# Wuziyi616/LEOD

Hardware: AMD Instinct MI355X
Metric: event-frames/sec/GPU (RVT-S train, Gen1 T=21) at 1/2/4/8 GPUs; mAP@0.5 parity (higher is better)
Workload: dtype fp16

## Files before the change

leod_amd/csrc/k_linear_wgrad.hip:

```cpp
#include "linear_common.hpp"
#include "wgrad_bf16.hpp"
#include "wgrad_dma.hpp"

LEOD_API long leod_workspace_bytes() { return (long)kWgwScratchBytes; }
LEOD_API int leod_set_workspace(void* ws, long bytes, hipStream_t stream) {
    if (ws && (bytes <= 0 || (reinterpret_cast<uintptr_t>(ws) & 15))) return LEOD_ERR_ARG;
    wgrad_wide_register_scratch(stream, ws, (size_t)(bytes > 0 ? bytes : 0));
    return LEOD_OK;
}

__global__ void leod_family_marker_kernel(int begin) { (void)begin; }
struct FamilyMarker {
    hipStream_t s; bool on;
    explicit FamilyMarker(hipStream_t st) : s(st) {
        static const bool env = getenv("LEOD_FAMILY_MARKERS") && atoi(getenv("LEOD_FAMILY_MARKERS"));
        on = env;
        if (on) hipLaunchKernelGGL(leod_family_marker_kernel, dim3(1), dim3(1), 0, s, 1);
    }
    ~FamilyMarker() { if (on) hipLaunchKernelGGL(leod_family_marker_kernel, dim3(1), dim3(1), 0, s, 0); }
};

enum : int { WGR_NONE = 0, WGR_DMA = 100, WGR_WIDE = 200, WGR_WGRADW = 300, WGR_LADDER = 400 };
static int wgrad_route(const XRows& xl, long lddy, int dyfmt, int M, int N, int K, bool dma = true) {
    const int xm = xl.x_mode();
    const bool x16 = xm == XM_BF16 || xm == XM_F16;
    if (x16 && (xl.stats || xl.x2)) return LEOD_ERR_ARG;
    if (dma && wgrad_dma_ok(xl, lddy, M, N, K, dyfmt)) return WGR_DMA + wgd_tile(N, K);
    if (use_wgrad_wide(xl, lddy, M, N, K, dyfmt)) return WGR_WIDE + wgrad_wide_combo(xl, N, K, dyfmt);
    if (x16) return LEOD_ERR_UNSUPPORTED;
    if (M <= 0) return WGR_NONE;
    if (!wgrad_rows16b_ok(lddy, N, K)) return LEOD_ERR_ARG;
// ... 98 lines not shown
```

leod_amd/csrc/wgrad_bf16.hpp:

```cpp
#pragma once

typedef unsigned u4_ __attribute__((ext_vector_type(4)));

__device__ __forceinline__ f2_ gelu_erf2(f2_ x) {
    const f2_ z = __builtin_elementwise_abs(x) * 0.70710678118654752440f;
    const f2_ d = z * 0.3275911f + 1.0f;
    const f2_ t = {fast_rcp(d.x), fast_rcp(d.y)};
    const f2_ poly = t * (0.254829592f + t * (-0.284496736f + t * (1.421413741f + t * (-1.453152027f + t * 1.061405429f))));
    const f2_ a = (z * z) * -1.4426950408889634f;
    const f2_ e = {__builtin_amdgcn_exp2f(a.x), __builtin_amdgcn_exp2f(a.y)};
    const f2_ ht = (0.5f * poly) * e;
    const f2_ cdf = {x.x >= 0.f ? 1.0f - ht.x : ht.x, x.y >= 0.f ? 1.0f - ht.y : ht.y};
    return x * cdf;
}
__device__ __forceinline__ unsigned pack_bf16x2(f2_ v) { return __builtin_bit_cast(unsigned, __builtin_convertvector(v, bf2_)); }

constexpr int wgw_row_groups(int slots_per_row) {
    int g = 1;
    while (2 * g * slots_per_row <= 256) g *= 2;
    return g;
}
template <int RG, int T, int BST>
__device__ __forceinline__ constexpr int wgw_slot_off(int e) {
    return RG >= 16 ? e * (RG / 16) * T * BST : (e % (16 / (RG < 16 ? RG : 16))) * RG * 16 + (e / (16 / (RG < 16 ? RG : 16))) * T * BST;
}

template <int TN, int TK, int RC, int MS = 1>
constexpr int wgw_lds_bytes() {
    return 2 * ((RC / 16) * (TN + TK) * 272) * 2 > (MS - 1) * 12 * 1024 ? 2 * ((RC / 16) * (TN + TK) * 272) * 2 : (MS - 1) * 12 * 1024;
}

template <int TN, int TK, int NWN, int NWK, int RC, int DYF, int XM, int OCC>
__global__ __launch_bounds__(256, OCC) void wgrad_wide_bf16_kernel(const void* __restrict__ dyv, long lddy, XRows xl, float* dW, long ldw,
                                                                    float* dbias, f4* __restrict__ part, int M, int N, int K, int dbg) {
    constexpr int WA = TN / NWN, WB = TK / NWK, MS = 4 / (NWN * NWK), KS = RC / 32;
    constexpr bool K16 = KS % MS != 0;
    constexpr int NSL = WA * WB + WA;
    static_assert((WA == 3 || WA == 6) && (WB == 3 || WB == 6) && WA * WB <= 18 && NWN * NWK * MS == 4 && (RC / 16) % MS == 0 &&
                  (MS == 1 || (WA == 3 && WB == 3)), "4 waves of 3 x 3, 6 x 3 or 3 x 6 tiles");
    constexpr int BST = 16 * 16 + 16;
    constexpr int DCW = DYF ? 8 : 4, XCW = XM >= XM_GELU16 ? 8 : 4;
    constexpr int DSPR = 16 * TN / DCW, XSPR = 16 * TK / XCW;
    constexpr int DRG = wgw_row_groups(DSPR) < RC ? wgw_row_groups(DSPR) : RC, XRG = wgw_row_groups(XSPR) < RC ? wgw_row_groups(XSPR) : RC;
    constexpr bool XG = XM == XM_GELU16;
    static_assert(!XG || (RC * XSPR) % 256 == 0, "whole slots per thread");
    constexpr int RN = RC / DRG, RK = XG ? RC * XSPR / 256 : RC / XRG;
    constexpr int SDY = (RC / 16) * TN * BST, SX = (RC / 16) * TK * BST;
    static_assert(DSPR * DRG == 192 && (XG || XSPR * XRG == 192), "three waves stage an operand");
    static_assert(2 * (SDY + SX) * 2 <= wgw_lds_bytes<TN, TK, RC, MS>(), "LDS size");
    extern __shared__ __attribute__((aligned(16))) unsigned short wg_smem[];
    const int tid = threadIdx.x, lane = tid & 63, wave = __builtin_amdgcn_readfirstlane(tid >> 6);
    const int i = lane & 15, q = lane >> 4;
    const int wn = wave % NWN, wk = (wave / NWN) % NWK, ws = wave / (NWN * NWK);
    const int n0 = blockIdx.y * TN * 16, k0 = blockIdx.z * TK * 16;
    const bool dact = wave < 3, xact = XG || wave >= 1;
    const int xt = tid - 64;
    const int dcs = tid % DSPR, drg = tid / DSPR, xcs = (xact ? xt : 0) % XSPR, xrg = (xact ? xt : 0) / XSPR;
// ... 186 lines not shown
    }
    __syncthreads();
    int buf = 0;
    for (; m0 < M; m0 += mstride) {
        const long mn = m0 + mstride;
        const bool more = mn < M;
        if (more) { if (mn + RC <= M) fetch(mn, FULL); else fetch(mn, TAILC); }
        if (!(dbg & 2)) mfma_chunk(buf);
        if (more) stash(mn, buf ^ 1);
        __syncthreads();
        buf ^= 1;
    }
    if constexpr (MS > 1) {
        f4* sred = reinterpret_cast<f4*>(wg_smem);
        if (ws > 0) {
#pragma unroll
            for (int a = 0; a < WA; ++a) {
#pragma unroll
                for (int b = 0; b < WB; ++b) sred[((ws - 1) * NSL + a * WB + b) * 64 + lane] = acc[a][b];
                sred[((ws - 1) * NSL + WA * WB + a) * 64 + lane] = bacc[a];
            }
        }
        __syncthreads();
        if (ws > 0) return;
#pragma unroll
        for (int o = 0; o < MS - 1; ++o)
#pragma unroll
            for (int a = 0; a < WA; ++a) {
#pragma unroll
                for (int b = 0; b < WB; ++b) acc[a][b] += sred[(o * NSL + a * WB + b) * 64 + lane];
                bacc[a] += sred[(o * NSL + WA * WB + a) * 64 + lane];
            }
    }
    if (dbg & 1) return;
    if constexpr (XM == XM_LN) {
#pragma unroll
        for (int b = 0; b < WB; ++b) {
            const int k = k0 + 16 * (wk * WB + b) + i;
            const float g = k < K ? xl.ln_w[k] : 0.f, sh = k < K ? xl.ln_b[k] : 0.f;
#pragma unroll
            for (int a = 0; a < WA; ++a)
#pragma unroll
                for (int r = 0; r < 4; ++r) acc[a][b][r] = fmaf(g, acc[a][b][r], sh * bacc[a][r]);
        }
    }
    const bool bias_out = dbias != nullptr && blockIdx.z == 0;
    if (part != nullptr) {
        constexpr int NW = NWN * NWK;
        const long tile = (long)blockIdx.y * gridDim.z + blockIdx.z, ntiles = (long)gridDim.y * gridDim.z;
        f4* dst = part + (((long)blockIdx.x * ntiles + tile) * NW + (wk * NWN + wn)) * (NSL * 64) + lane;
#pragma unroll
        for (int a = 0; a < WA; ++a) {
#pragma unroll
            for (int b = 0; b < WB; ++b) dst[(a * WB + b) * 64] = acc[a][b];
            if (bias_out && a % NWK == wk) dst[(WA * WB + a) * 64] = bacc[a];
        }
        return;
    }
#pragma unroll
    for (int b = 0; b < WB; ++b) {
        const int k = k0 + 16 * (wk * WB + b) + i;
#pragma unroll
        for (int a = 0; a < WA; ++a)
#pragma unroll
            for (int r = 0; r < 4; ++r) {
                const int n = n0 + 16 * (wn * WA + a) + 4 * q + r;
                if (n < N && k < K) atomicAdd(dW + (long)n * ldw + k, acc[a][b][r]);
            }
    }
    if (bias_out && i == 0) {
#pragma unroll
        for (int a = 0; a < WA; ++a)
            if (a % NWK == wk) {
#pragma unroll
                for (int r = 0; r < 4; ++r) {
                    const int n = n0 + 16 * (wn * WA + a) + 4 * q + r;
                    if (n < N) atomicAdd(dbias + n, bacc[a][r]);
                }
            }
    }
}

template <int TN, int TK, int NWN, int NWK>
__global__ __launch_bounds__(256) void wgrad_wide_reduce_kernel(const f4* __restrict__ part, int gx, int ny, int nz, int per, float* dW, long ldw,
                                                                float* dbias, int N, int K) {
    constexpr int NW = NWN * NWK, WA = TN / NWN, WB = TK / NWK, NT9 = WA * WB, NSL = NT9 + WA;
    const long O = (long)ny * nz * NW * NSL * 64;
    const long o = (long)blockIdx.x * 256 + threadIdx.x;
    if (o >= O) return;
    const int lane = (int)(o & 63), t = (int)((o >> 6) % NSL), w = (int)((o / (64 * NSL)) % NW), tile = (int)(o / (64 * NSL * NW));
    const int ty = tile / nz, tz = tile - ty * nz, wn = w % NWN, wk = w / NWN, i = lane & 15, q = lane >> 4;
    if (t >= NT9 && !(dbias != nullptr && tz == 0 && (t - NT9) % NWK == wk && i == 0)) return;
    const int g0 = blockIdx.y * per, g1 = min(gx, g0 + per);
    f4 s0 = zero4(), s1 = zero4(), s2 = zero4(), s3 = zero4();
    const f4* p = part + (long)g0 * O + o;
    int g = g0;
    f4 s4 = zero4(), s5 = zero4(), s6 = zero4(), s7 = zero4();
    for (; g + 8 <= g1; g += 8, p += 8 * O) {
        s0 += p[0]; s1 += p[O]; s2 += p[2 * O]; s3 += p[3 * O]; s4 += p[4 * O]; s5 += p[5 * O]; s6 += p[6 * O]; s7 += p[7 * O];
    }
    for (; g + 4 <= g1; g += 4, p += 4 * O) { s0 += p[0]; s1 += p[O]; s2 += p[2 * O]; s3 += p[3 * O]; }
    for (; g < g1; ++g, p += O) s0 += p[0];
    const f4 v = ((s0 + s1) + (s2 + s3)) + ((s4 + s5) + (s6 + s7));
    const bool single = gridDim.y == 1;
    if (t < NT9) {
        const int a = t / WB, b = t - a * WB;
        const int k = tz * TK * 16 + 16 * (wk * WB + b) + i;
#pragma unroll
        for (int r = 0; r < 4; ++r) {
            const int n = ty * TN * 16 + 16 * (wn * WA + a) + 4 * q + r;
            if (n < N && k < K) {
                float* d = dW + (long)n * ldw + k;
                if (single) *d += v[r]; else atomicAdd(d, v[r]);
            }
        }
    } else {
#pragma unroll
        for (int r = 0; r < 4; ++r) {
            const int n = ty * TN * 16 + 16 * (wn * WA + (t - NT9)) + 4 * q + r;
            if (n < N) { if (single) dbias[n] += v[r]; else atomicAdd(dbias + n, v[r]); }
        }
    }
}

#include <mutex>
#include <unordered_map>
struct WgwScratch { void* p = nullptr; size_t bytes = 0; };
static inline std::unordered_map<hipStream_t, WgwScratch>& wgw_scratch_map() { static std::unordered_map<hipStream_t, WgwScratch> m; return m; }
static inline std::mutex& wgw_scratch_mutex() { static std::mutex m; return m; }
constexpr size_t kWgwScratchBytes = (size_t)768 << 20;
static inline void wgrad_wide_register_scratch(hipStream_t s, void* p, size_t bytes) {
    std::lock_guard<std::mutex> lock(wgw_scratch_mutex());
    WgwScratch& e = wgw_scratch_map()[s];
    e.p = p; e.bytes = p ? bytes : 0;
}
static inline f4* wgrad_wide_scratch(hipStream_t s, size_t bytes) {
    std::lock_guard<std::mutex> lock(wgw_scratch_mutex());
    WgwScratch& e = wgw_scratch_map()[s];
    if (e.bytes >= bytes) return reinterpret_cast<f4*>(e.p);
    hipStreamCaptureStatus cs = hipStreamCaptureStatusNone;
    if (hipStreamIsCapturing(s, &cs) != hipSuccess || cs != hipStreamCaptureStatusNone) { (void)hipGetLastError(); return nullptr; }
    void* nb = nullptr;
    const size_t want = bytes < kWgwScratchBytes ? kWgwScratchBytes : bytes;
    if (hipMalloc(&nb, want) != hipSuccess) { (void)hipGetLastError(); return nullptr; }
    e.p = nb; e.bytes = want;
    return reinterpret_cast<f4*>(nb);
}

template <int TN, int TK, int NWN, int NWK, int RC, int DYF, int XM, int OCC>
static inline int launch_wgrad_wide_cfg(const void* dy, long lddy, const XRows& xl, float* dW, long ldw, float* dbias,
                                        int M, int N, int K, hipStream_t s) {
    constexpr int dbg = 0;
    constexpr int LDS = wgw_lds_bytes<TN, TK, RC, 4 / (NWN * NWK)>();
    const int tiles = cdiv(N, TN * 16) * cdiv(K, TK * 16), chunks = cdiv(M, RC);
    const int wgs = M <= 60000 ? 384 : OCC * 256;
    int gx = max(1, min(chunks / 2, wgs / tiles));
    if (gx >= 16) gx &= ~7;
    dim3 grid(gx, cdiv(N, TN * 16), cdiv(K, TK * 16));
    auto kern = wgrad_wide_bf16_kernel<TN, TK, NWN, NWK, RC, DYF, XM, OCC>;
    static bool attr_set = false;
    if (!attr_set) { hipFuncSetAttribute(reinterpret_cast<const void*>(kern), hipFuncAttributeMaxDynamicSharedMemorySize, LDS); attr_set = true; }
    constexpr int NW = NWN * NWK, NSL = (TN / NWN) * (TK / NWK) + TN / NWN;
    const long O = (long)tiles * NW * NSL * 64;
    f4* part = gx > 1 ? wgrad_wide_scratch(s, (size_t)gx * O * sizeof(f4)) : nullptr;
    hipLaunchKernelGGL(kern, grid, dim3(256), LDS, s, dy, lddy, xl, dW, ldw, dbias, part, M, N, K, dbg);
    if (part != nullptr && !(dbg & 1)) {
        const int ob = (int)cdiv(O, 256);
        int groups = max(1, min(gx, 512 / ob));
        const int per = cdiv(gx, groups);
        groups = cdiv(gx, per);
        hipLaunchKernelGGL((wgrad_wide_reduce_kernel<TN, TK, NWN, NWK>), dim3(ob, groups), dim3(256), 0, s, part, gx, (int)grid.y, (int)grid.z, per,
                           dW, ldw, dbias, N, K);
    }
    return leod_launch_status();
}

static inline int wgrad_wide_combo(const XRows& xl, int N, int K, int dyfmt) {
    const int xm = xl.x_mode();
    if (xm == XM_F16) {
        if (dyfmt) return 0;
        if (N <= 48 && K <= 48) return 14;
        if (K <= 48 || N <= 48) return 0;
        return (K % 192 == 0 && N >= 96) ? 16 : 15;
    }
    const bool f32_rows = !dyfmt && xm == XM_ROWS, f32_gelu = !dyfmt && xm == XM_GELU16, f32_bf16 = !dyfmt && xm == XM_BF16;
    const bool b16_rows = dyfmt && xm == XM_ROWS, b16_ln = dyfmt && xm == XM_LN;
    if (N <= 48 && K <= 48) return f32_rows ? 1 : f32_bf16 ? 8 : 0;
    if (K <= 48) return b16_ln ? 2 : 0;
    if (N <= 48) return f32_gelu ? 3 : 0;
    if (N % 192 == 0 && K >= 96 && (b16_ln || b16_rows)) return b16_ln ? 10 : 11;
    if (K % 192 == 0 && N >= 96 && (f32_gelu || f32_bf16)) return f32_gelu ? 12 : 13;
    return f32_rows ? 4 : b16_ln ? 5 : f32_gelu ? 6 : b16_rows ? 7 : f32_bf16 ? 9 : 0;
}
static inline bool use_wgrad_wide(const XRows& xl, long lddy, int M, int N, int K, int dyfmt) {
    if (leod_precision() != 1 || M < 8192) return false;
    const int xm = xl.x_mode();
// ... 31 lines not shown
```

leod_amd/csrc/wgrad_dma.hpp:

```cpp
#pragma once

struct Prep16 {
    const void* src; long ld;
    const float* src2; long ld2; int C1;
    const float* stats;
    unsigned short* dst;
    int C, mode;
};
enum Prep16Mode : int { P16_NONE = -1, P16_F32 = 0, P16_LN = 1 , P16_GELU16 = 2, P16_F16 = 3, P16_CONCAT = 4  };
static inline int prep16_mode(int xm, bool concat) {
    if (xm_is_mfma_operand(xm)) return P16_NONE;
    return xm == XM_LN ? P16_LN : xm == XM_GELU16 ? P16_GELU16 : xm == XM_F16 ? P16_F16 : concat ? P16_CONCAT : P16_F32;
}

struct Prep16Group { Prep16 a[4]; Prep16 b[4]; };
__global__ __launch_bounds__(256) void wgrad_prep16_kernel(Prep16Group grp, int M) {
    const Prep16& p = blockIdx.y ? grp.b[blockIdx.z] : grp.a[blockIdx.z];
    if (p.mode < 0) return;
    const int C8 = p.C >> 3;
    const long it = (long)blockIdx.x * 256 + threadIdx.x;
    if (it >= (long)M * C8) return;
    const long m = it / C8;
    const int c = (int)(it - m * C8) << 3;
    f4 lo, hi;
// ... 6 lines not shown
    } else {
        const float* s = (p.mode == 4 && c >= p.C1) ? p.src2 + m * p.ld2 + (c - p.C1) : reinterpret_cast<const float*>(p.src) + m * p.ld + c;
        lo = ld4(s); hi = ld4(s + 4);
        if (p.mode == 1) {
            const f2_ st = *reinterpret_cast<const f2_*>(p.stats + 2 * m);
            lo = (lo - st.x) * st.y; hi = (hi - st.x) * st.y;
        }
    }
    const u4_ o = {pack_bf16x2(f2_{lo.x, lo.y}), pack_bf16x2(f2_{lo.z, lo.w}), pack_bf16x2(f2_{hi.x, hi.y}), pack_bf16x2(f2_{hi.z, hi.w})};
    *reinterpret_cast<u4_*>(p.dst + m * p.C + c) = o;
}

__device__ __forceinline__ void wgd_dma16(const void* gsrc, unsigned lds_dst) {
    unsigned keep;
    asm volatile("s_mov_b32 %0, m0\n\ts_mov_b32 m0, %2\n\ts_nop 0\n\tglobal_load_lds_dwordx4 %1, off\n\ts_mov_b32 m0, %0"
                 : "=&s"(keep) : "v"(gsrc), "s"(lds_dst) : "memory");
}
template <int N> __device__ __forceinline__ void wgd_wait_vm() { asm volatile("s_waitcnt vmcnt(%0)" :: "n"(N) : "memory"); }

template <int T, int RC, int NS> constexpr int wgd_lds_bytes() { return NS * 2 * (RC / 16) * T * 256 * 2; }
template <int T, int RC, int NS> constexpr int wgd_occupancy() { return wgd_lds_bytes<T, RC, NS>() <= 52 * 1024 ? 3 : wgd_lds_bytes<T, RC, NS>() <= 80 * 1024 ? 2 : 1; }

struct WgdProb {
    const unsigned short* A; long lda; const unsigned short* B; long ldb; const float* ln_w; const float* ln_b; float* dbias_flag; f4* part;
    int cpw, gx, ny, nz, N, K, blk0;
};
struct WgdGroup { WgdProb p[4]; int n; };
template <int T, int RC, int NS, bool LN>
__global__ __launch_bounds__(256, ((wgd_occupancy<T, RC, NS>()) >= 2 ? 2 : 1)) void wgrad_dma_kernel(WgdGroup grp, int chunks, int dbg) {
    int pk = 0;
    for (int k = 1; k < grp.n; ++k) if ((int)blockIdx.x >= grp.p[k].blk0) pk = k;
    const WgdProb& pr = grp.p[pk];
    const unsigned short* __restrict__ A = pr.A; const unsigned short* __restrict__ B = pr.B; const long lda = pr.lda, ldb = pr.ldb;
    const float* __restrict__ ln_w = pr.ln_w; const float* __restrict__ ln_b = pr.ln_b; float* dbias_flag = pr.dbias_flag; f4* __restrict__ part = pr.part;
    const int cpw = pr.cpw, gx = pr.gx, ny = pr.ny, nz = pr.nz, K = pr.K;
    const int bid = (int)blockIdx.x - pr.blk0;
    const bool ln = LN && ln_w != nullptr;
    constexpr int WA = T / 2, WB = T / 2, NWN = 2, NWK = 2, RB = RC / 16, KS = RC / 32;
    constexpr int BLK = 256;
    constexpr int SA = RB * T * BLK, SLOT = 2 * SA;
    constexpr int NI = SLOT * 2 / 1024, IPW = NI / 4;
    static_assert(NI % 4 == 0 && RC % 32 == 0, "whole instructions per wave");
    constexpr int NSL = WA * WB + WA;
    extern __shared__ __attribute__((aligned(1024))) unsigned short wd_smem[];
    const int tid = threadIdx.x, lane = tid & 63, wave = __builtin_amdgcn_readfirstlane(tid >> 6);
    const int i = lane & 15, q = lane >> 4;
    const int wn = wave % NWN, wk = wave / NWN;
    const int ntl = ny * nz;
    int tl, bx;
    if ((gx & 7) == 0) { const int xcd = bid & 7, sj = bid >> 3; tl = sj % ntl; bx = (sj / ntl) * 8 + xcd; }
    else { bx = bid % gx; tl = bid / gx; }
    const int by = tl / nz, bz = tl - by * nz;
    const int n0 = by * T * 16, k0 = bz * T * 16;
    const int c0 = bx * cpw, c1 = min(chunks, c0 + cpw);
    const int nch = c1 - c0;
    static_assert(IPW % 2 == 0, "the first half of a wave's instructions fills the dY part, the second half the X part");
    const char* src[IPW];
    const long stepA = (long)RC * lda * 2, stepB = (long)RC * ldb * 2;
#pragma unroll
    for (int j = 0; j < IPW; ++j) {
        const int t = wave + 4 * j;
        const int blk = 2 * t + (lane >> 5), r = (lane & 31) >> 1, half = lane & 1;
        const bool isb = j >= IPW / 2;
        const int b = isb ? blk - RB * T : blk;
        const int rb = b / T, cb = b - rb * T;
        const long ld = isb ? ldb : lda;
        const int col = (isb ? k0 : n0) + cb * 16 + half * 8;
        src[j] = reinterpret_cast<const char*>(isb ? B : A) + (((long)c0 * RC + rb * 16 + r) * ld + col) * 2;
    }
    const unsigned lds0 = __builtin_amdgcn_readfirstlane((unsigned)(size_t)wd_smem);
    auto issue = [&](int slot) {
#pragma unroll
        for (int j = 0; j < IPW; ++j) {
            wgd_dma16(src[j], __builtin_amdgcn_readfirstlane(lds0 + (unsigned)(slot * SLOT * 2 + (wave + 4 * j) * 1024)));
            src[j] += j >= IPW / 2 ? stepB : stepA;
        }
    };
    const bool bias_out = dbias_flag != nullptr && bz == 0;
    const bool bias_any = ln || bias_out;
    f4 acc[WA][WB], bacc[WA];
#pragma unroll
    for (int a = 0; a < WA; ++a) {
        bacc[a] = zero4();
#pragma unroll
        for (int b = 0; b < WB; ++b) acc[a][b] = zero4();
    }
    const s8v ones = {0x3F80, 0x3F80, 0x3F80, 0x3F80, 0x3F80, 0x3F80, 0x3F80, 0x3F80};
    typedef __attribute__((address_space(3))) s4 lds_s4;
    const int loff = (4 * q + (i >> 2)) * 16 + 4 * (i & 3);
    auto mfma_chunk = [&](int slot) {
        const unsigned short* pdy = wd_smem + slot * SLOT + (wn * WA) * BLK + loff;
        const unsigned short* px = wd_smem + slot * SLOT + SA + (wk * WB) * BLK + loff;
#pragma unroll
        for (int ks = 0; ks < KS; ++ks) {
            const int st = 2 * ks;
            s8v pa[WA], pb[WB];
#pragma unroll
            for (int a = 0; a < WA; ++a) {
                const s4 lo = __builtin_amdgcn_ds_read_tr16_b64_v4i16((lds_s4*)(pdy + (st * T + a) * BLK));
                const s4 hi = __builtin_amdgcn_ds_read_tr16_b64_v4i16((lds_s4*)(pdy + ((st + 1) * T + a) * BLK));
                pa[a] = __builtin_shufflevector(lo, hi, 0, 1, 2, 3, 4, 5, 6, 7);
// ... 25 lines not shown
        if (c + NS - 1 < nch && !(dbg & 2)) issue((c + NS - 1) % NS);
        if (!(dbg & 1)) mfma_chunk(c % NS);
    }
    if (ln) {
#pragma unroll
        for (int b = 0; b < WB; ++b) {
            const int k = k0 + 16 * (wk * WB + b) + i;
            const float g = k < K ? ln_w[k] : 0.f, sh = k < K ? ln_b[k] : 0.f;
#pragma unroll
            for (int a = 0; a < WA; ++a)
#pragma unroll
                for (int r = 0; r < 4; ++r) acc[a][b][r] = fmaf(g, acc[a][b][r], sh * bacc[a][r]);
        }
    }
    constexpr int NW = NWN * NWK;
    const long tile = (long)by * nz + bz, ntiles = ntl;
    f4* dst = part + (((long)bx * ntiles + tile) * NW + (wk * NWN + wn)) * (NSL * 64) + lane;
#pragma unroll
    for (int a = 0; a < WA; ++a) {
#pragma unroll
        for (int b = 0; b < WB; ++b) dst[(a * WB + b) * 64] = acc[a][b];
        if (bias_out && a % NWK == wk) dst[(WA * WB + a) * 64] = bacc[a];
    }
}

constexpr int kWgdRC = 64;
constexpr size_t kWgdOperandBytes = (size_t)600 << 20;

static inline int wgd_tile(int N, int K) {
    if (N % 96 == 0 && K % 96 == 0) return 6;
    if (N % 128 == 0 && K % 128 == 0) return 8;
    if (N % 64 == 0 && K % 64 == 0) return 4;
    return 0;
}
static inline bool wgrad_dma_ok(const XRows& xl, long lddy, int M, int N, int K, int dyfmt) {
    if (leod_precision() != 1 || M < 8192 || (M % kWgdRC) || N < 64 || K < 64) return false;
    const int T = wgd_tile(N, K);
    if (!T) return false;
    const int xm = xl.x_mode();
    if ((lddy & 7) || (xl.ld & 7)) return false;
    if (xl.x2 && (xm != XM_ROWS || (xl.K1 & 7) || (xl.ld2 & 7))) return false;
    const size_t need = (size_t)M * ((dyfmt ? 0 : N) + (xm_is_mfma_operand(xm) ? 0 : K)) * 2;
    if (need > kWgdOperandBytes) return false;
    if (M > (T == 6 ? 60000 : 400000)) return false;
    if (!dyfmt && xm != XM_BF16 && xm != XM_GELU16 && (long)N * K < 200000) return false;
    return true;
}

struct WgrProb { const f4* part; float* dW; float* dbias; long ldw; int gx, ny, nz, per, N, K, ob, groups; };
struct WgrGroup { WgrProb p[4]; };
template <int T>
__global__ __launch_bounds__(256) void wgrad_dma_reduce_kernel(WgrGroup grp) {
    const WgrProb& pr = grp.p[blockIdx.z];
    if ((int)blockIdx.x >= pr.ob || (int)blockIdx.y >= pr.groups) return;
    constexpr int NWN = 2, NWK = 2, NW = 4, WA = T / 2, WB = T / 2, NT9 = WA * WB, NSL = NT9 + WA;
    const int gx = pr.gx, nz = pr.nz, per = pr.per, N = pr.N, K = pr.K;
    float* dW = pr.dW; float* dbias = pr.dbias; const long ldw = pr.ldw;
    const long O = (long)pr.ny * nz * NW * NSL * 64;
    const long o = (long)blockIdx.x * 256 + threadIdx.x;
    if (o >= O) return;
    const int lane = (int)(o & 63), t = (int)((o >> 6) % NSL), w = (int)((o / (64 * NSL)) % NW), tile = (int)(o / (64 * NSL * NW));
    const int ty = tile / nz, tz = tile - ty * nz, wn = w % NWN, wk = w / NWN, i = lane & 15, q = lane >> 4;
    if (t >= NT9 && !(dbias != nullptr && tz == 0 && (t - NT9) % NWK == wk && i == 0)) return;
    const int g0 = blockIdx.y * per, g1 = min(gx, g0 + per);
    f4 s0 = zero4(), s1 = zero4(), s2 = zero4(), s3 = zero4(), s4 = zero4(), s5 = zero4(), s6 = zero4(), s7 = zero4();
    const f4* p = pr.part + (long)g0 * O + o;
    int g = g0;
    for (; g + 8 <= g1; g += 8, p += 8 * O) {
        s0 += p[0]; s1 += p[O]; s2 += p[2 * O]; s3 += p[3 * O]; s4 += p[4 * O]; s5 += p[5 * O]; s6 += p[6 * O]; s7 += p[7 * O];
    }
    for (; g + 4 <= g1; g += 4, p += 4 * O) { s0 += p[0]; s1 += p[O]; s2 += p[2 * O]; s3 += p[3 * O]; }
    for (; g < g1; ++g, p += O) s0 += p[0];
    const f4 v = ((s0 + s1) + (s2 + s3)) + ((s4 + s5) + (s6 + s7));
    const bool single = pr.groups == 1;
    if (t < NT9) {
        const int a = t / WB, b = t - a * WB;
        const int k = tz * T * 16 + 16 * (wk * WB + b) + i;
#pragma unroll
        for (int r = 0; r < 4; ++r) {
            const int n = ty * T * 16 + 16 * (wn * WA + a) + 4 * q + r;
            if (n < N && k < K) {
                float* d = dW + (long)n * ldw + k;
                if (single) *d += v[r]; else atomicAdd(d, v[r]);
            }
        }
    } else {
#pragma unroll
        for (int r = 0; r < 4; ++r) {
            const int n = ty * T * 16 + 16 * (wn * WA + (t - NT9)) + 4 * q + r;
            if (n < N) { if (single) dbias[n] += v[r]; else atomicAdd(dbias + n, v[r]); }
        }
    }
}

struct WgdHostProb { const void* dy; long lddy; XRows xl; float* dW; long ldw; float* dbias; int N, K, dyfmt; };

template <int T, int RC, int NS>
static inline int launch_wgrad_dma_group_t(int n, const WgdHostProb* hp, int M, hipStream_t s) {
    constexpr int TW = T * 16;
    constexpr int LDS = wgd_lds_bytes<T, RC, NS>();
    constexpr int dbg = 0;
    constexpr int NW = 4, NSL = (T / 2) * (T / 2) + T / 2;
    const int chunks = M / RC;
    const int target = 256 * wgd_occupancy<T, RC, NS>();
    int total_tiles = 0;
    for (int k = 0; k < n; ++k) total_tiles += (hp[k].N / TW) * (hp[k].K / TW);
    WgdGroup g{};
    WgrGroup rg{};
    Prep16Group pg{};
    size_t off = 0, offs_part[4], offs_a[4], offs_b[4];
    int blk = 0, obmax = 0, grmax = 0, c8max = 0;
    bool any_ln = false, any_prep = false;
    for (int k = 0; k < n; ++k) {
        const WgdHostProb& h = hp[k];
        const int xm = h.xl.x_mode();
        const int tiles = (h.N / TW) * (h.K / TW);
        int gx = max(1, min(chunks / NS, target / total_tiles));
        if (gx >= 8) gx &= ~7;
        const int cpw = cdiv(chunks, gx);
        if (gx < 8) gx = cdiv(chunks, cpw);
        const long O = (long)tiles * NW * NSL * 64;
        offs_part[k] = off; off += ((size_t)gx * O * sizeof(f4) + 1023) & ~(size_t)1023;
        offs_a[k] = off; off += h.dyfmt ? 0 : (((size_t)M * h.N * 2 + 1023) & ~(size_t)1023);
        offs_b[k] = off; off += xm_is_mfma_operand(xm) ? 0 : (((size_t)M * h.K * 2 + 1023) & ~(size_t)1023);
        g.p[k].cpw = cpw; g.p[k].gx = gx; g.p[k].ny = h.N / TW; g.p[k].nz = h.K / TW; g.p[k].N = h.N; g.p[k].K = h.K; g.p[k].blk0 = blk;
        blk += gx * tiles;
        const int ob = (int)cdiv(O, 256);
        int groups = max(1, min(gx, 512 / ob));
        const int per = cdiv(gx, groups);
        groups = cdiv(gx, per);
        rg.p[k] = WgrProb{nullptr, h.dW, h.dbias, h.ldw, gx, h.N / TW, h.K / TW, per, h.N, h.K, ob, groups};
        obmax = max(obmax, ob); grmax = max(grmax, groups);
        any_ln = any_ln || xm == XM_LN;
    }
    g.n = n;
    char* ws = reinterpret_cast<char*>(wgrad_wide_scratch(s, off + 4096));
    if (!ws) return LEOD_ERR_UNSUPPORTED;
    for (int k = 0; k < n; ++k) {
        const WgdHostProb& h = hp[k];
        const int xm = h.xl.x_mode();
        f4* part = reinterpret_cast<f4*>(ws + offs_part[k]);
        unsigned short* a16 = reinterpret_cast<unsigned short*>(ws + offs_a[k]);
        unsigned short* b16 = reinterpret_cast<unsigned short*>(ws + offs_b[k]);
        Prep16 pa{}, pb{};
        pa.mode = pb.mode = P16_NONE;
        if (!h.dyfmt) pa = Prep16{h.dy, h.lddy, nullptr, 0, 0, nullptr, a16, h.N, P16_F32};
        if (!xm_is_mfma_operand(xm)) pb = Prep16{h.xl.x, h.xl.ld, h.xl.x2, h.xl.ld2, h.xl.x2 ? h.xl.K1 : h.K, h.xl.stats, b16, h.K,
                                                 prep16_mode(xm, h.xl.x2 != nullptr)};
        pg.a[k] = pa; pg.b[k] = pb;
        if (pa.mode >= 0) { any_prep = true; c8max = max(c8max, h.N / 8); }
        if (pb.mode >= 0) { any_prep = true; c8max = max(c8max, h.K / 8); }
        g.p[k].A = h.dyfmt ? reinterpret_cast<const unsigned short*>(h.dy) : a16;
        g.p[k].lda = h.dyfmt ? h.lddy : h.N;
        g.p[k].B = xm_is_mfma_operand(xm) ? reinterpret_cast<const unsigned short*>(h.xl.x) : b16;
        g.p[k].ldb = xm_is_mfma_operand(xm) ? h.xl.ld : h.K;
        g.p[k].ln_w = xm == XM_LN ? h.xl.ln_w : nullptr; g.p[k].ln_b = xm == XM_LN ? h.xl.ln_b : nullptr;
        g.p[k].dbias_flag = h.dbias; g.p[k].part = part;
        rg.p[k].part = part;
    }
    for (int k = n; k < 4; ++k) { pg.a[k].mode = pg.b[k].mode = P16_NONE; }
    if (any_prep) hipLaunchKernelGGL(wgrad_prep16_kernel, dim3(cdiv((long)M * c8max, 256), 2, n), dim3(256), 0, s, pg, M);
    if (any_ln) {
        auto kern = wgrad_dma_kernel<T, RC, NS, true>;
        static bool attr_set = false;
        if (!attr_set) { hipFuncSetAttribute(reinterpret_cast<const void*>(kern), hipFuncAttributeMaxDynamicSharedMemorySize, LDS); attr_set = true; }
        hipLaunchKernelGGL(kern, dim3(blk), dim3(256), LDS, s, g, chunks, dbg);
    } else {
        auto kern = wgrad_dma_kernel<T, RC, NS, false>;
        static bool attr_set = false;
        if (!attr_set) { hipFuncSetAttribute(reinterpret_cast<const void*>(kern), hipFuncAttributeMaxDynamicSharedMemorySize, LDS); attr_set = true; }
        hipLaunchKernelGGL(kern, dim3(blk), dim3(256), LDS, s, g, chunks, dbg);
    }
    hipLaunchKernelGGL(wgrad_dma_reduce_kernel<T>, dim3(obmax, grmax, n), dim3(256), 0, s, rg);
    return leod_launch_status();
}
template <int T, int RC, int NS>
static inline int launch_wgrad_dma_t(const void* dy, long lddy, const XRows& xl, float* dW, long ldw, float* dbias,
                                     int M, int N, int K, hipStream_t s, int dyfmt) {
    const WgdHostProb h{dy, lddy, xl, dW, ldw, dbias, N, K, dyfmt};
    return launch_wgrad_dma_group_t<T, RC, NS>(1, &h, M, s);
}
static inline int launch_wgrad_dma(int tile, const void* dy, long lddy, const XRows& xl, float* dW, long ldw, float* dbias,
                                   int M, int N, int K, hipStream_t s, int dyfmt) {
    switch (tile) {
        case 6: return launch_wgrad_dma_t<6, 64, 3>(dy, lddy, xl, dW, ldw, dbias, M, N, K, s, dyfmt);
        case 8: return launch_wgrad_dma_t<8, 64, 2>(dy, lddy, xl, dW, ldw, dbias, M, N, K, s, dyfmt);
        case 4: return launch_wgrad_dma_t<4, 64, 3>(dy, lddy, xl, dW, ldw, dbias, M, N, K, s, dyfmt);
    }
    return LEOD_ERR_ARG;
}
```

leod_amd/ops.py:

```python
from typing import Optional, Sequence, Tuple

import ctypes

import torch

from ._lib import lib, check, LeodHipError, DevPtr

F32 = torch.float32


_LIB = None


def _l():
    global _LIB
    if _LIB is None:
        _LIB = lib()
    return _LIB


try:
    _raw_stream = torch._C._cuda_getCurrentRawStream
except AttributeError:
    _raw_stream = None
# ... 1287 lines not shown
    def dump(self, path: str):
        check(_l().leod_plan_dump(self.handle, path.encode()), 'plan_dump')

    def close(self):
        if getattr(self, 'handle', 0):
            _l().leod_plan_destroy(self.handle)
            self.handle = 0
        self.graph = None

    def __del__(self):
        try:
            self.close()
        except Exception:
            pass

_PROBE = None


class KernelProbe:

    def __init__(self, targets=('linear_wgrad', 'linear_gemm'), kernel_names=None, families=True):
        global _PROBE, _LIB
        self.targets = tuple(targets)
        self.kernel_names = kernel_names or {'linear_wgrad': 'wgrad_wide_bf16_kernel + wgrad_wide_reduce_kernel (bf16 mode) / wgradw_kernel<.., XRows> (f32 mode)',
                                             'linear_gemm': 'rowstream* / gemm_lds_kernel / gemm_wide_bf16_kernel (Linear forward + dgrad)'}
        self.step = 0
        self.events = {t: [] for t in self.targets}
        self.fam_events = {}
        self.calls = []
        self.real_lib = _l()
        if families:
            _LIB = _ProbedLib(self.real_lib, self)
        _PROBE = self

    def mark_step(self):
        self.step += 1

    @property
    def steps(self):
        return max(self.step, 1)

    def begin(self, target, nbytes, flops=0.0, rows=None, nbytes16=None):
        e0, e1 = torch.cuda.Event(enable_timing=True), torch.cuda.Event(enable_timing=True)
        e0.record()
        self.events[target].append((self.step, e0, e1, nbytes, flops, nbytes if nbytes16 is None else nbytes16, rows))
        return e1

# ... 106 lines not shown
```

Baseline: 11310.

## Fuse split-K partial reduction into wgrad kernels via last-block atomic counters

Removes the separate wgrad_wide_reduce and wgrad_dma_reduce kernel launches. Each block writes its partials, then bumps a per-group, per-tile counter held in a zeroed region at the start of the workspace. The last block of a group sums the partials and adds them into dW and dbias. This drops a launch per wgrad call and lets the reduction overlap with blocks that are still computing. In exchange it adds a serial tail on the last block, fences and an atomic counter, and needs counters that reset themselves, plus an extra memset when the workspace is registered.

```diff
diff --git a/leod_amd/csrc/k_linear_wgrad.hip b/leod_amd/csrc/k_linear_wgrad.hip
--- a/leod_amd/csrc/k_linear_wgrad.hip
+++ b/leod_amd/csrc/k_linear_wgrad.hip
@@ -5,8 +5,7 @@
 LEOD_API long leod_workspace_bytes() { return (long)kWgwScratchBytes; }
 LEOD_API int leod_set_workspace(void* ws, long bytes, hipStream_t stream) {
     if (ws && (bytes <= 0 || (reinterpret_cast<uintptr_t>(ws) & 15))) return LEOD_ERR_ARG;
-    wgrad_wide_register_scratch(stream, ws, (size_t)(bytes > 0 ? bytes : 0));
-    return LEOD_OK;
+    return wgrad_wide_register_scratch(stream, ws, (size_t)(bytes > 0 ? bytes : 0)) ? LEOD_OK : LEOD_ERR_LAUNCH;
 }
 
 __global__ void leod_family_marker_kernel(int begin) { (void)begin; }
diff --git a/leod_amd/csrc/wgrad_bf16.hpp b/leod_amd/csrc/wgrad_bf16.hpp
--- a/leod_amd/csrc/wgrad_bf16.hpp
+++ b/leod_amd/csrc/wgrad_bf16.hpp
@@ -30,9 +30,89 @@
     return 2 * ((RC / 16) * (TN + TK) * 272) * 2 > (MS - 1) * 12 * 1024 ? 2 * ((RC / 16) * (TN + TK) * 272) * 2 : (MS - 1) * 12 * 1024;
 }
 
+template <int TN, int TK, int NWN, int NWK, int JUMAX = 2>
+__device__ __forceinline__ void wgrad_fused_reduce_tail(const f4* __restrict__ part, long O, int* cnt, int bx, int gx, int per, int ntiles, int tile,
+                                                        int ty, int tz, float* dW, long ldw, float* dbias, int N, int K, unsigned* flag) {
+    constexpr int NW = NWN * NWK, WA = TN / NWN, WB = TK / NWK, NT9 = WA * WB, NSL = NT9 + WA, TSZ = NW * NSL * 64, NIT = TSZ / 256;
+    constexpr int JU = (NIT % 2 == 0 && JUMAX >= 2) ? 2 : 1;
+    static_assert(TSZ % 256 == 0, "whole elements per thread");
+    const int tid = threadIdx.x;
+    const int grp = bx / per, g0 = grp * per, g1 = min(gx, g0 + per);
+    asm volatile("s_waitcnt vmcnt(0)" ::: "memory");
+    __syncthreads();
+    if (tid == 0) {
+        __builtin_amdgcn_fence(__ATOMIC_RELEASE, "agent");
+        asm volatile("s_waitcnt vmcnt(0)" ::: "memory");
+        int* c = cnt + (long)grp * ntiles + tile;
+        const int old = __hip_atomic_fetch_add(c, 1, __ATOMIC_RELAXED, __HIP_MEMORY_SCOPE_AGENT);
+        const bool last = old == g1 - g0 - 1;
+        if (last) {
+            __hip_atomic_store(c, 0, __ATOMIC_RELAXED, __HIP_MEMORY_SCOPE_AGENT);
+            __builtin_amdgcn_fence(__ATOMIC_ACQUIRE, "agent");
+            asm volatile("s_waitcnt vmcnt(0)" ::: "memory");
+        }
+        *flag = last ? 1u : 0u;
+    }
+    __syncthreads();
+    if (*flag == 0u) return;
+    const bool single = per >= gx;
+    const f4* base = part + (long)g0 * O + (long)tile * TSZ + tid;
+#pragma unroll 1
+    for (int j = 0; j < NIT; j += JU) {
+        f4 sm[JU][8];
+#pragma unroll
+        for (int u = 0; u < JU; ++u)
+#pragma unroll
+            for (int e = 0; e < 8; ++e) sm[u][e] = zero4();
+        const f4* p = base + j * 256;
+        int g = g0;
+        for (; g + 8 <= g1; g += 8, p += 8 * O) {
+#pragma unroll
+            for (int u = 0; u < JU; ++u)
+#pragma unroll
+                for (int e = 0; e < 8; ++e) sm[u][e] += p[e * O + u * 256];
+        }
+        for (; g + 4 <= g1; g += 4, p += 4 * O) {
+#pragma unroll
+            for (int u = 0; u < JU; ++u)
+#pragma unroll
+                for (int e = 0; e < 4; ++e) sm[u][e] += p[e * O + u * 256];
+        }
+        for (; g < g1; ++g, p += O) {
+#pragma unroll
+            for (int u = 0; u < JU; ++u) sm[u][0] += p[u * 256];
+        }
+#pragma unroll
+        for (int u = 0; u < JU; ++u) {
+            const f4 v = ((sm[u][0] + sm[u][1]) + (sm[u][2] + sm[u][3])) + ((sm[u][4] + sm[u][5]) + (sm[u][6] + sm[u][7]));
+            const int o = tid + (j + u) * 256;
+            const int lane = o & 63, t = (o >> 6) % NSL, w = o / (64 * NSL);
+            const int wn = w % NWN, wk = w / NWN, i = lane & 15, q = lane >> 4;
+            if (t < NT9) {
+                const int a = t / WB, b = t - a * WB;
+                const int k = tz * TK * 16 + 16 * (wk * WB + b) + i;
+#pragma unroll
+                for (int r = 0; r < 4; ++r) {
+                    const int n = ty * TN * 16 + 16 * (wn * WA + a) + 4 * q + r;
+                    if (n < N && k < K) {
+                        float* d = dW + (long)n * ldw + k;
+                        if (single) *d += v[r]; else atomicAdd(d, v[r]);
+                    }
+                }
+            } else if (dbias != nullptr && tz == 0 && (t - NT9) % NWK == wk && i == 0) {
+#pragma unroll
+                for (int r = 0; r < 4; ++r) {
+                    const int n = ty * TN * 16 + 16 * (wn * WA + (t - NT9)) + 4 * q + r;
+                    if (n < N) { if (single) dbias[n] += v[r]; else atomicAdd(dbias + n, v[r]); }
+                }
+            }
+        }
+    }
+}
+
 template <int TN, int TK, int NWN, int NWK, int RC, int DYF, int XM, int OCC>
 __global__ __launch_bounds__(256, OCC) void wgrad_wide_bf16_kernel(const void* __restrict__ dyv, long lddy, XRows xl, float* dW, long ldw,
-                                                                    float* dbias, f4* __restrict__ part, int M, int N, int K, int dbg) {
+                                                                    float* dbias, f4* __restrict__ part, int* cnt, int per, int M, int N, int K, int dbg) {
     constexpr int WA = TN / NWN, WB = TK / NWK, MS = 4 / (NWN * NWK), KS = RC / 32;
     constexpr bool K16 = KS % MS != 0;
     constexpr int NSL = WA * WB + WA;
@@ -265,7 +345,8 @@
             }
         }
         __syncthreads();
-        if (ws > 0) return;
+        if (ws > 0 && part == nullptr) return;
+        if (ws == 0) {
 #pragma unroll
         for (int o = 0; o < MS - 1; ++o)
 #pragma unroll
@@ -274,6 +355,7 @@
                 for (int b = 0; b < WB; ++b) acc[a][b] += sred[(o * NSL + a * WB + b) * 64 + lane];
                 bacc[a] += sred[(o * NSL + WA * WB + a) * 64 + lane];
             }
+        }
     }
     if (dbg & 1) return;
     if constexpr (XM == XM_LN) {
@@ -290,14 +372,18 @@
     const bool bias_out = dbias != nullptr && blockIdx.z == 0;
     if (part != nullptr) {
         constexpr int NW = NWN * NWK;
-        const long tile = (long)blockIdx.y * gridDim.z + blockIdx.z, ntiles = (long)gridDim.y * gridDim.z;
-        f4* dst = part + (((long)blockIdx.x * ntiles + tile) * NW + (wk * NWN + wn)) * (NSL * 64) + lane;
-#pragma unroll
-        for (int a = 0; a < WA; ++a) {
-#pragma unroll
-            for (int b = 0; b < WB; ++b) dst[(a * WB + b) * 64] = acc[a][b];
-            if (bias_out && a % NWK == wk) dst[(WA * WB + a) * 64] = bacc[a];
-        }
+        const int tile = blockIdx.y * gridDim.z + blockIdx.z, ntiles = gridDim.y * gridDim.z;
+        if (MS == 1 || ws == 0) {
+            f4* dst = part + (((long)blockIdx.x * ntiles + tile) * NW + (wk * NWN + wn)) * (NSL * 64) + lane;
+#pragma unroll
+            for (int a = 0; a < WA; ++a) {
+#pragma unroll
+                for (int b = 0; b < WB; ++b) dst[(a * WB + b) * 64] = acc[a][b];
+                if (bias_out && a % NWK == wk) dst[(WA * WB + a) * 64] = bacc[a];
+            }
+        }
+        wgrad_fused_reduce_tail<TN, TK, NWN, NWK, (OCC >= 4 ? 1 : 2)>(part, (long)ntiles * (NW * NSL * 64), cnt, blockIdx.x, gridDim.x, per, ntiles, tile, blockIdx.y,
+                                                  blockIdx.z, dW, ldw, dbias, N, K, reinterpret_cast<unsigned*>(wg_smem));
         return;
     }
 #pragma unroll
@@ -321,48 +407,6 @@
                     if (n < N) atomicAdd(dbias + n, bacc[a][r]);
                 }
             }
-    }
-}
-
-template <int TN, int TK, int NWN, int NWK>
-__global__ __launch_bounds__(256) void wgrad_wide_reduce_kernel(const f4* __restrict__ part, int gx, int ny, int nz, int per, float* dW, long ldw,
-                                                                float* dbias, int N, int K) {
-    constexpr int NW = NWN * NWK, WA = TN / NWN, WB = TK / NWK, NT9 = WA * WB, NSL = NT9 + WA;
-    const long O = (long)ny * nz * NW * NSL * 64;
-    const long o = (long)blockIdx.x * 256 + threadIdx.x;
-    if (o >= O) return;
-    const int lane = (int)(o & 63), t = (int)((o >> 6) % NSL), w = (int)((o / (64 * NSL)) % NW), tile = (int)(o / (64 * NSL * NW));
-    const int ty = tile / nz, tz = tile - ty * nz, wn = w % NWN, wk = w / NWN, i = lane & 15, q = lane >> 4;
-    if (t >= NT9 && !(dbias != nullptr && tz == 0 && (t - NT9) % NWK == wk && i == 0)) return;
-    const int g0 = blockIdx.y * per, g1 = min(gx, g0 + per);
-    f4 s0 = zero4(), s1 = zero4(), s2 = zero4(), s3 = zero4();
-    const f4* p = part + (long)g0 * O + o;
-    int g = g0;
-    f4 s4 = zero4(), s5 = zero4(), s6 = zero4(), s7 = zero4();
-    for (; g + 8 <= g1; g += 8, p += 8 * O) {
-        s0 += p[0]; s1 += p[O]; s2 += p[2 * O]; s3 += p[3 * O]; s4 += p[4 * O]; s5 += p[5 * O]; s6 += p[6 * O]; s7 += p[7 * O];
-    }
-    for (; g + 4 <= g1; g += 4, p += 4 * O) { s0 += p[0]; s1 += p[O]; s2 += p[2 * O]; s3 += p[3 * O]; }
-    for (; g < g1; ++g, p += O) s0 += p[0];
-    const f4 v = ((s0 + s1) + (s2 + s3)) + ((s4 + s5) + (s6 + s7));
-    const bool single = gridDim.y == 1;
-    if (t < NT9) {
-        const int a = t / WB, b = t - a * WB;
-        const int k = tz * TK * 16 + 16 * (wk * WB + b) + i;
-#pragma unroll
-        for (int r = 0; r < 4; ++r) {
-            const int n = ty * TN * 16 + 16 * (wn * WA + a) + 4 * q + r;
-            if (n < N && k < K) {
-                float* d = dW + (long)n * ldw + k;
-                if (single) *d += v[r]; else atomicAdd(d, v[r]);
-            }
-        }
-    } else {
-#pragma unroll
-        for (int r = 0; r < 4; ++r) {
-            const int n = ty * TN * 16 + 16 * (wn * WA + (t - NT9)) + 4 * q + r;
-            if (n < N) { if (single) dbias[n] += v[r]; else atomicAdd(dbias + n, v[r]); }
-        }
     }
 }
 
@@ -372,22 +416,33 @@
 static inline std::unordered_map<hipStream_t, WgwScratch>& wgw_scratch_map() { static std::unordered_map<hipStream_t, WgwScratch> m; return m; }
 static inline std::mutex& wgw_scratch_mutex() { static std::mutex m; return m; }
 constexpr size_t kWgwScratchBytes = (size_t)768 << 20;
-static inline void wgrad_wide_register_scratch(hipStream_t s, void* p, size_t bytes) {
+constexpr size_t kWgwCounterBytes = (size_t)64 << 10;
+constexpr int kWgwCounters = (int)(kWgwCounterBytes / sizeof(int));
+static inline bool wgrad_wide_register_scratch(hipStream_t s, void* p, size_t bytes) {
     std::lock_guard<std::mutex> lock(wgw_scratch_mutex());
     WgwScratch& e = wgw_scratch_map()[s];
+    if (p && hipMemsetAsync(p, 0, bytes < kWgwCounterBytes ? bytes : kWgwCounterBytes, s) != hipSuccess) {
+        (void)hipGetLastError();
+        e.p = nullptr; e.bytes = 0;
+        return false;
+    }
     e.p = p; e.bytes = p ? bytes : 0;
-}
-static inline f4* wgrad_wide_scratch(hipStream_t s, size_t bytes) {
+    return true;
+}
+struct WgwBuf { int* cnt; f4* part; };
+static inline WgwBuf wgrad_wide_scratch(hipStream_t s, size_t bytes) {
     std::lock_guard<std::mutex> lock(wgw_scratch_mutex());
     WgwScratch& e = wgw_scratch_map()[s];
-    if (e.bytes >= bytes) return reinterpret_cast<f4*>(e.p);
+    auto split = [](void* p) { return WgwBuf{reinterpret_cast<int*>(p), reinterpret_cast<f4*>(reinterpret_cast<char*>(p) + kWgwCounterBytes)}; };
+    if (e.bytes >= bytes + kWgwCounterBytes) return split(e.p);
     hipStreamCaptureStatus cs = hipStreamCaptureStatusNone;
-    if (hipStreamIsCapturing(s, &cs) != hipSuccess || cs != hipStreamCaptureStatusNone) { (void)hipGetLastError(); return nullptr; }
+    if (hipStreamIsCapturing(s, &cs) != hipSuccess || cs != hipStreamCaptureStatusNone) { (void)hipGetLastError(); return WgwBuf{nullptr, nullptr}; }
     void* nb = nullptr;
-    const size_t want = bytes < kWgwScratchBytes ? kWgwScratchBytes : bytes;
-    if (hipMalloc(&nb, want) != hipSuccess) { (void)hipGetLastError(); return nullptr; }
+    const size_t want = bytes + kWgwCounterBytes < kWgwScratchBytes ? kWgwScratchBytes : bytes + kWgwCounterBytes;
+    if (hipMalloc(&nb, want) != hipSuccess) { (void)hipGetLastError(); return WgwBuf{nullptr, nullptr}; }
+    if (hipMemsetAsync(nb, 0, kWgwCounterBytes, s) != hipSuccess) { (void)hipGetLastError(); (void)hipFree(nb); return WgwBuf{nullptr, nullptr}; }
     e.p = nb; e.bytes = want;
-    return reinterpret_cast<f4*>(nb);
+    return split(nb);
 }
 
 template <int TN, int TK, int NWN, int NWK, int RC, int DYF, int XM, int OCC>
@@ -405,16 +460,13 @@
     if (!attr_set) { hipFuncSetAttribute(reinterpret_cast<const void*>(kern), hipFuncAttributeMaxDynamicSharedMemorySize, LDS); attr_set = true; }
     constexpr int NW = NWN * NWK, NSL = (TN / NWN) * (TK / NWK) + TN / NWN;
     const long O = (long)tiles * NW * NSL * 64;
-    f4* part = gx > 1 ? wgrad_wide_scratch(s, (size_t)gx * O * sizeof(f4)) : nullptr;
-    hipLaunchKernelGGL(kern, grid, dim3(256), LDS, s, dy, lddy, xl, dW, ldw, dbias, part, M, N, K, dbg);
-    if (part != nullptr && !(dbg & 1)) {
-        const int ob = (int)cdiv(O, 256);
-        int groups = max(1, min(gx, 512 / ob));
-        const int per = cdiv(gx, groups);
-        groups = cdiv(gx, per);
-        hipLaunchKernelGGL((wgrad_wide_reduce_kernel<TN, TK, NWN, NWK>), dim3(ob, groups), dim3(256), 0, s, part, gx, (int)grid.y, (int)grid.z, per,
-                           dW, ldw, dbias, N, K);
-    }
+    const int ob = (int)cdiv(O, 256);
+    int groups = max(1, min(gx, 512 / ob));
+    const int per = cdiv(gx, groups);
+    groups = cdiv(gx, per);
+    WgwBuf ws{nullptr, nullptr};
+    if (gx > 1 && (long)groups * tiles <= kWgwCounters) ws = wgrad_wide_scratch(s, (size_t)gx * O * sizeof(f4));
+    hipLaunchKernelGGL(kern, grid, dim3(256), LDS, s, dy, lddy, xl, dW, ldw, dbias, ws.part, ws.cnt, per, M, N, K, dbg);
     return leod_launch_status();
 }
 
diff --git a/leod_amd/csrc/wgrad_dma.hpp b/leod_amd/csrc/wgrad_dma.hpp
--- a/leod_amd/csrc/wgrad_dma.hpp
+++ b/leod_amd/csrc/wgrad_dma.hpp
@@ -52,8 +52,9 @@
 template <int T, int RC, int NS> constexpr int wgd_occupancy() { return wgd_lds_bytes<T, RC, NS>() <= 52 * 1024 ? 3 : wgd_lds_bytes<T, RC, NS>() <= 80 * 1024 ? 2 : 1; }
 
 struct WgdProb {
-    const unsigned short* A; long lda; const unsigned short* B; long ldb; const float* ln_w; const float* ln_b; float* dbias_flag; f4* part;
-    int cpw, gx, ny, nz, N, K, blk0;
+    const unsigned short* A; long lda; const unsigned short* B; long ldb; const float* ln_w; const float* ln_b; float* dbias; f4* part;
+    float* dW; long ldw; int* cnt;
+    int cpw, gx, ny, nz, N, K, blk0, per;
 };
 struct WgdGroup { WgdProb p[4]; int n; };
 template <int T, int RC, int NS, bool LN>
@@ -62,7 +63,7 @@
     for (int k = 1; k < grp.n; ++k) if ((int)blockIdx.x >= grp.p[k].blk0) pk = k;
     const WgdProb& pr = grp.p[pk];
     const unsigned short* __restrict__ A = pr.A; const unsigned short* __restrict__ B = pr.B; const long lda = pr.lda, ldb = pr.ldb;
-    const float* __restrict__ ln_w = pr.ln_w; const float* __restrict__ ln_b = pr.ln_b; float* dbias_flag = pr.dbias_flag; f4* __restrict__ part = pr.part;
+    const float* __restrict__ ln_w = pr.ln_w; const float* __restrict__ ln_b = pr.ln_b; float* dbias = pr.dbias; f4* __restrict__ part = pr.part;
     const int cpw = pr.cpw, gx = pr.gx, ny = pr.ny, nz = pr.nz, K = pr.K;
     const int bid = (int)blockIdx.x - pr.blk0;
     const bool ln = LN && ln_w != nullptr;
@@ -106,7 +107,7 @@
             src[j] += j >= IPW / 2 ? stepB : stepA;
         }
     };
-    const bool bias_out = dbias_flag != nullptr && bz == 0;
+    const bool bias_out = dbias != nullptr && bz == 0;
     const bool bias_any = ln || bias_out;
     f4 acc[WA][WB], bacc[WA];
 #pragma unroll
@@ -178,10 +179,13 @@
         for (int b = 0; b < WB; ++b) dst[(a * WB + b) * 64] = acc[a][b];
         if (bias_out && a % NWK == wk) dst[(WA * WB + a) * 64] = bacc[a];
     }
+    wgrad_fused_reduce_tail<T, T, NWN, NWK>(part, ntiles * (NW * NSL * 64), pr.cnt, bx, gx, pr.per, ntl, (int)tile, by, bz, pr.dW, pr.ldw, dbias,
+                                            pr.N, K, reinterpret_cast<unsigned*>(wd_smem));
 }
 
 constexpr int kWgdRC = 64;
 constexpr size_t kWgdOperandBytes = (size_t)600 << 20;
+static_assert(kWgwCounterBytes + ((size_t)64 << 20) + kWgdOperandBytes + 4096 <= kWgwScratchBytes, "workspace layout");
 
 static inline int wgd_tile(int N, int K) {
     if (N % 96 == 0 && K % 96 == 0) return 6;
@@ -203,52 +207,6 @@
     return true;
 }
 
-struct WgrProb { const f4* part; float* dW; float* dbias; long ldw; int gx, ny, nz, per, N, K, ob, groups; };
-struct WgrGroup { WgrProb p[4]; };
-template <int T>
-__global__ __launch_bounds__(256) void wgrad_dma_reduce_kernel(WgrGroup grp) {
-    const WgrProb& pr = grp.p[blockIdx.z];
-    if ((int)blockIdx.x >= pr.ob || (int)blockIdx.y >= pr.groups) return;
-    constexpr int NWN = 2, NWK = 2, NW = 4, WA = T / 2, WB = T / 2, NT9 = WA * WB, NSL = NT9 + WA;
-    const int gx = pr.gx, nz = pr.nz, per = pr.per, N = pr.N, K = pr.K;
-    float* dW = pr.dW; float* dbias = pr.dbias; const long ldw = pr.ldw;
-    const long O = (long)pr.ny * nz * NW * NSL * 64;
-    const long o = (long)blockIdx.x * 256 + threadIdx.x;
-    if (o >= O) return;
-    const int lane = (int)(o & 63), t = (int)((o >> 6) % NSL), w = (int)((o / (64 * NSL)) % NW), tile = (int)(o / (64 * NSL * NW));
-    const int ty = tile / nz, tz = tile - ty * nz, wn = w % NWN, wk = w / NWN, i = lane & 15, q = lane >> 4;
-    if (t >= NT9 && !(dbias != nullptr && tz == 0 && (t - NT9) % NWK == wk && i == 0)) return;
-    const int g0 = blockIdx.y * per, g1 = min(gx, g0 + per);
-    f4 s0 = zero4(), s1 = zero4(), s2 = zero4(), s3 = zero4(), s4 = zero4(), s5 = zero4(), s6 = zero4(), s7 = zero4();
-    const f4* p = pr.part + (long)g0 * O + o;
-    int g = g0;
-    for (; g + 8 <= g1; g += 8, p += 8 * O) {
-        s0 += p[0]; s1 += p[O]; s2 += p[2 * O]; s3 += p[3 * O]; s4 += p[4 * O]; s5 += p[5 * O]; s6 += p[6 * O]; s7 += p[7 * O];
-    }
-    for (; g + 4 <= g1; g += 4, p += 4 * O) { s0 += p[0]; s1 += p[O]; s2 += p[2 * O]; s3 += p[3 * O]; }
-    for (; g < g1; ++g, p += O) s0 += p[0];
-    const f4 v = ((s0 + s1) + (s2 + s3)) + ((s4 + s5) + (s6 + s7));
-    const bool single = pr.groups == 1;
-    if (t < NT9) {
-        const int a = t / WB, b = t - a * WB;
-        const int k = tz * T * 16 + 16 * (wk * WB + b) + i;
-#pragma unroll
-        for (int r = 0; r < 4; ++r) {
-            const int n = ty * T * 16 + 16 * (wn * WA + a) + 4 * q + r;
-            if (n < N && k < K) {
-                float* d = dW + (long)n * ldw + k;
-                if (single) *d += v[r]; else atomicAdd(d, v[r]);
-            }
-        }
-    } else {
-#pragma unroll
-        for (int r = 0; r < 4; ++r) {
-            const int n = ty * T * 16 + 16 * (wn * WA + (t - NT9)) + 4 * q + r;
-            if (n < N) { if (single) dbias[n] += v[r]; else atomicAdd(dbias + n, v[r]); }
-        }
-    }
-}
-
 struct WgdHostProb { const void* dy; long lddy; XRows xl; float* dW; long ldw; float* dbias; int N, K, dyfmt; };
 
 template <int T, int RC, int NS>
@@ -262,10 +220,9 @@
     int total_tiles = 0;
     for (int k = 0; k < n; ++k) total_tiles += (hp[k].N / TW) * (hp[k].K / TW);
     WgdGroup g{};
-    WgrGroup rg{};
     Prep16Group pg{};
     size_t off = 0, offs_part[4], offs_a[4], offs_b[4];
-    int blk = 0, obmax = 0, grmax = 0, c8max = 0;
+    int blk = 0, c8max = 0, ncnt = 0, cnt0[4];
     bool any_ln = false, any_prep = false;
     for (int k = 0; k < n; ++k) {
         const WgdHostProb& h = hp[k];
@@ -285,12 +242,15 @@
         int groups = max(1, min(gx, 512 / ob));
         const int per = cdiv(gx, groups);
         groups = cdiv(gx, per);
-        rg.p[k] = WgrProb{nullptr, h.dW, h.dbias, h.ldw, gx, h.N / TW, h.K / TW, per, h.N, h.K, ob, groups};
-        obmax = max(obmax, ob); grmax = max(grmax, groups);
+        g.p[k].per = per; g.p[k].dW = h.dW; g.p[k].ldw = h.ldw;
+        cnt0[k] = ncnt;
+        if ((long)ncnt + (long)groups * tiles > kWgwCounters) return LEOD_ERR_UNSUPPORTED;
+        ncnt += groups * tiles;
         any_ln = any_ln || xm == XM_LN;
     }
     g.n = n;
-    char* ws = reinterpret_cast<char*>(wgrad_wide_scratch(s, off + 4096));
+    const WgwBuf wb = wgrad_wide_scratch(s, off + 4096);
+    char* ws = reinterpret_cast<char*>(wb.part);
     if (!ws) return LEOD_ERR_UNSUPPORTED;
     for (int k = 0; k < n; ++k) {
         const WgdHostProb& h = hp[k];
@@ -311,8 +271,7 @@
         g.p[k].B = xm_is_mfma_operand(xm) ? reinterpret_cast<const unsigned short*>(h.xl.x) : b16;
         g.p[k].ldb = xm_is_mfma_operand(xm) ? h.xl.ld : h.K;
         g.p[k].ln_w = xm == XM_LN ? h.xl.ln_w : nullptr; g.p[k].ln_b = xm == XM_LN ? h.xl.ln_b : nullptr;
-        g.p[k].dbias_flag = h.dbias; g.p[k].part = part;
-        rg.p[k].part = part;
+        g.p[k].dbias = h.dbias; g.p[k].part = part; g.p[k].cnt = wb.cnt + cnt0[k];
     }
     for (int k = n; k < 4; ++k) { pg.a[k].mode = pg.b[k].mode = P16_NONE; }
     if (any_prep) hipLaunchKernelGGL(wgrad_prep16_kernel, dim3(cdiv((long)M * c8max, 256), 2, n), dim3(256), 0, s, pg, M);
@@ -327,7 +286,6 @@
         if (!attr_set) { hipFuncSetAttribute(reinterpret_cast<const void*>(kern), hipFuncAttributeMaxDynamicSharedMemorySize, LDS); attr_set = true; }
         hipLaunchKernelGGL(kern, dim3(blk), dim3(256), LDS, s, g, chunks, dbg);
     }
-    hipLaunchKernelGGL(wgrad_dma_reduce_kernel<T>, dim3(obmax, grmax, n), dim3(256), 0, s, rg);
     return leod_launch_status();
 }
 template <int T, int RC, int NS>
diff --git a/leod_amd/ops.py b/leod_amd/ops.py
--- a/leod_amd/ops.py
+++ b/leod_amd/ops.py
@@ -1333,7 +1333,7 @@
     def __init__(self, targets=('linear_wgrad', 'linear_gemm'), kernel_names=None, families=True):
         global _PROBE, _LIB
         self.targets = tuple(targets)
-        self.kernel_names = kernel_names or {'linear_wgrad': 'wgrad_wide_bf16_kernel + wgrad_wide_reduce_kernel (bf16 mode) / wgradw_kernel<.., XRows> (f32 mode)',
+        self.kernel_names = kernel_names or {'linear_wgrad': 'wgrad_wide_bf16_kernel / wgrad_dma_kernel (16-bit modes) / wgradw_kernel<.., XRows> (f32 mode)',
                                              'linear_gemm': 'rowstream* / gemm_lds_kernel / gemm_wide_bf16_kernel (Linear forward + dgrad)'}
         self.step = 0
         self.events = {t: [] for t in self.targets}
```

Measured after the change: 10600. 6.3% lower.
